# Aikku93/ulc-codec

Hardware: AMD Instinct MI355X
Metric: encode+decode Msamples/s at BlockSize=2048 stereo (channel-samples through encode+decode, VBR -50, 32 blocks per stream per call) (higher is better)
Workload: dtype f32; 1 GPU; vbr50 (configs[1] encode, configs[2] decode): Batch=4096 independent 44.1 kHz stereo streams/GPU x 32 blocks, BlockSize=2048, VBR -50; step = encode then decode; config=vbr50, mode=both, streams_per_gpu=4096, block_size=2048, channels=2, parallelism=batch split over 1 GPU(s), no collective on the data path

## Files before the change

### ulc-codec_amd/csrc/ulcx_enc_wc.hip

```cpp
#include "ulcx_enc_dev.h"

template <typename IN> __device__ __forceinline__ float2 wc_energy_at(const UlcxEncCtx &c, int s, int t) {
    float ehp = 0.0f, ebp = 0.0f;
    if (c.C == 2) {
        float2 a = smp_ld2<IN>(c, s, t - 1), b = smp_ld2<IN>(c, s, t), d = smp_ld2<IN>(c, s, t + 1);
        float m0 = (a.x + a.y) * 0.5f, m1 = (b.x + b.y) * 0.5f, m2 = (d.x + d.y) * 0.5f;
        float s0 = (a.x - a.y) * 0.5f, s1 = (b.x - b.y) * 0.5f, s2 = (d.x - d.y) * 0.5f;
        float hp = -m0 + 2 * m1 - m2, bp = -m0 + m2;
        ehp += hp * hp; ebp += bp * bp;
        hp = -s0 + 2 * s1 - s2; bp = -s0 + s2;
        ehp += hp * hp; ebp += bp * bp;
    } else {
        for (int ch = 0; ch < c.C; ch++) {
            float t0 = ms_sample<IN>(c, s, t - 1, ch), t1 = ms_sample<IN>(c, s, t, ch), t2 = ms_sample<IN>(c, s, t + 1, ch);
            float hp = -t0 + 2 * t1 - t2;
            float bp = -t0 + t2;
            ehp += hp * hp;
            ebp += bp * bp;
        }
    }
    return make_float2(sqrtf(ehp), sqrtf(ebp));
}

template <typename IN>
__global__ __launch_bounds__(WG) void k_wc_energy(UlcxEncCtx c, int k0, int k1) {
    __shared__ float2 tile[64][65];
    int tiles_t = ((k1 - k0) * c.BS) / 64;
    int sg = blockIdx.x / tiles_t, tt = blockIdx.x % tiles_t + (k0 * c.BS) / 64;
    int lane = threadIdx.x & 63, wv = __builtin_amdgcn_readfirstlane(threadIdx.x >> 6);
    int r = tt * 64 + lane;
    int t = r - c.BS / 2;
#pragma unroll 4
    for (int sl = wv; sl < 64; sl += 4) {
        int s = sg * 64 + sl;
        tile[lane][sl] = (s < c.B) ? wc_energy_at<IN>(c, s, t) : make_float2(0.0f, 0.0f);
    }
    __syncthreads();
    float *dst = (float *)c.env + envq_idx(c, sg * 64, tt * 16);
    for (int ql = wv; ql < 16; ql += 4) {
        const float2 a0 = tile[4 * ql][lane], a1 = tile[4 * ql + 1][lane], a2 = tile[4 * ql + 2][lane], a3 = tile[4 * ql + 3][lane];
        float4 *o = (float4 *)(dst + (size_t)ql * 512 + lane * 4);
        wc_st(o, make_float4(a0.x, a1.x, a2.x, a3.x));
        wc_st(o + 64, make_float4(a0.y, a1.y, a2.y, a3.y));
    }
}

__global__ __launch_bounds__(64) void k_wc_forward(UlcxEncCtx c, int k0, int k1) {
    __builtin_amdgcn_s_setprio(3);
    int gl = blockIdx.x * 64 + threadIdx.x;
    int s = gl >> 1, f = gl & 1;
    bool live = s < c.B;
    float4 *v = (float4 *)((float *)c.env + envq_idx(c, live ? s : 0, k0 * c.BS / 4) + f * 256);
    float env = live ? c.wcs[s].tf[f] : 0.0f;
    float cc = f ? c.cBP : c.cHP;
    const int nq = (k1 - k0) * c.BS / 4;
    constexpr int U = 2, D = 8;
    constexpr int QS = 512 / 4;
    const float4 *rp = v;
    float4 *wp = v;
    float4 x[D][U];
#pragma unroll
    for (int g = 0; g < D - 1; g++) {
#pragma unroll
        for (int j = 0; j < U; j++) x[g][j] = wc_ld(rp + (size_t)j * QS);
        rp += U * QS;
    }
    for (int i = 0; i < nq; i += D * U) {
#pragma unroll
        for (int g = 0; g < D; g++) {
            const bool more = (i + (g + D - 1) * U) < nq;
            const float4 *lp = more ? rp : v;
#pragma unroll
            for (int j = 0; j < U; j++) x[(g + D - 1) % D][j] = wc_ld(lp + (size_t)j * QS);
            rp += U * QS;
#pragma unroll
            for (int j = 0; j < U; j++) {
                float4 q = x[g][j];
                float d;
                d = q.x - env; env += d * cc; q.x = env;
                d = q.y - env; env += d * cc; q.y = env;
                d = q.z - env; env += d * cc; q.z = env;
                d = q.w - env; env += d * cc; q.w = env;
                x[g][j] = q;
            }
            if (live) {
#pragma unroll
                for (int j = 0; j < U; j++) wc_st(wp + (size_t)j * QS, x[g][j]);
            }
            wp += U * QS;
        }
    }
    if (live) c.wcs[s].tf[f] = env;
}

__device__ __forceinline__ float2 wc_energy_stereo(float2 a, float2 b, float2 d) {
    float m0 = (a.x + a.y) * 0.5f, m1 = (b.x + b.y) * 0.5f, m2 = (d.x + d.y) * 0.5f;
    float s0 = (a.x - a.y) * 0.5f, s1 = (b.x - b.y) * 0.5f, s2 = (d.x - d.y) * 0.5f;
    float ehp = 0.0f, ebp = 0.0f;
    float hp = -m0 + 2 * m1 - m2, bp = -m0 + m2;
    ehp += hp * hp; ebp += bp * bp;
    hp = -s0 + 2 * s1 - s2; bp = -s0 + s2;
    ehp += hp * hp; ebp += bp * bp;
    return make_float2(sqrtf(ehp), sqrtf(ebp));
}

template <int NW, typename IN>
__global__ __launch_bounds__(NW * 64) void k_wc_ef(UlcxEncCtx c, int k0, int k1) {
    extern __shared__ float efs[];
    float *ring = efs;
    int *flags = (int *)(ring + EF_RT * EF_TILE_FLOATS);
    const int wv = __builtin_amdgcn_readfirstlane(threadIdx.x >> 6), lane = threadIdx.x & 63;
    const int s0 = blockIdx.x * EF_SPW;
    const int nT = (k1 - k0) * c.BS / 64;
    constexpr int NP = NW - 1, NS = (EF_SPW + NP - 1) / NP;
    if (threadIdx.x < NW) flags[threadIdx.x] = 0;
    __syncthreads();
    if (wv > 0) {
        const int p = wv - 1;
        if (p >= EF_SPW) {
            if (lane == 0) __atomic_store_n(&flags[p], 0x7ffffff0, __ATOMIC_RELEASE);
            return;
        }
#ifndef EF_AHEAD
#define EF_AHEAD 3
#endif
        float2 A[EF_AHEAD][NS][3];
        const IN *sbase[NS];
#pragma unroll
        for (int i = 0; i < NS; i++) {
            const int s = s0 + p + NP * i;
            const int sc = ((p + NP * i < EF_SPW) && (s < c.B)) ? s : 0;
            sbase[i] = pcm_base<IN>(c) + (size_t)sc * c.K * c.BS * 2 + 2 * lane;
        }
        auto issue = [&](float2 (&A)[NS][3], int j) {
            const int t0 = (k0 * c.BS + j * 64) - c.BS / 2;
            const int t = t0 + lane;
#pragma unroll
            for (int i = 0; i < NS; i++) {
                const int s = s0 + p + NP * i;
                const bool on = (p + NP * i < EF_SPW) && (s < c.B);
                const int sc = on ? s : 0;
                if (t0 >= 1) {
                    const IN *q = sbase[i] + 2 * (ptrdiff_t)t0;
                    A[i][0] = ld2(q - 2); A[i][1] = ld2(q); A[i][2] = ld2(q + 2);
                } else { A[i][0] = smp_ld2<IN>(c, sc, t - 1); A[i][1] = smp_ld2<IN>(c, sc, t); A[i][2] = smp_ld2<IN>(c, sc, t + 1); }
            }
        };
        auto step = [&](float2 (&A)[NS][3], int j) {
            float2 v[NS];
#pragma unroll
            for (int i = 0; i < NS; i++) v[i] = wc_energy_stereo(A[i][0], A[i][1], A[i][2]);
            if (j + EF_AHEAD < nT) issue(A, j + EF_AHEAD);
            while (j >= __atomic_load_n(&flags[NP], __ATOMIC_ACQUIRE) + EF_RT) __builtin_amdgcn_s_sleep(4);
            float *tile = ring + (j % EF_RT) * EF_TILE_FLOATS;
#pragma unroll
            for (int i = 0; i < NS; i++) {
                const int sl = p + NP * i;
                if (sl < EF_SPW) {
                    const bool on = s0 + sl < c.B;
                    tile[(sl * 2 + 0) * EF_TS + lane] = on ? v[i].x : 0.0f;
                    tile[(sl * 2 + 1) * EF_TS + lane] = on ? v[i].y : 0.0f;
                }
            }
            __builtin_amdgcn_fence(__ATOMIC_RELEASE, "workgroup");
            if (lane == 0) __atomic_store_n(&flags[p], j + 1, __ATOMIC_RELEASE);
        };
#pragma unroll
        for (int a = 0; a < EF_AHEAD; a++) if (a < nT) issue(A[a], a);
        for (int j = 0; j < nT; j += EF_AHEAD) {
#pragma unroll
            for (int a = 0; a < EF_AHEAD; a++) if (j + a < nT) step(A[a], j + a);
        }
        return;
    }
    if (lane >= 2 * EF_SPW) return;
    __builtin_amdgcn_s_setprio(3);
    const int s = s0 + (lane >> 1), f = lane & 1;
    const bool live = s < c.B;
    float env = live ? c.wcs[s].tf[f] : 0.0f;
    const float cc = f ? c.cBP : c.cHP;
    constexpr int QS = 512 / 4;
    char *wq[4];
#pragma unroll
    for (int k = 0; k < 4; k++) wq[k] = (char *)((float *)c.env + envq_idx(c, s, k0 * c.BS / 4) + f * 256) + k * 8192 + 4096;
    for (int j = 0; j < nT; j++) {
        for (;;) {
            int m = (lane < NP) ? __atomic_load_n(&flags[lane], __ATOMIC_ACQUIRE) : 0x7fffffff;
            if (__all(m > j)) break;
            __builtin_amdgcn_s_sleep(1);
        }
        const float4 *row = (const float4 *)(ring + (j % EF_RT) * EF_TILE_FLOATS + lane * EF_TS);
        float4 x[16];
#pragma unroll
        for (int q = 0; q < 16; q++) x[q] = row[q];
        if (lane == 0) __atomic_store_n(&flags[NP], j + 1, __ATOMIC_RELEASE);
#pragma unroll
        for (int q = 0; q < 16; q++) {
            float4 v = x[q];
            float d;
            d = v.x - env; env += d * cc; v.x = env;
            d = v.y - env; env += d * cc; v.y = env;
            d = v.z - env; env += d * cc; v.z = env;
            d = v.w - env; env += d * cc; v.w = env;
            wc_st((float4 *)(wq[q >> 2] + ((q & 3) * 2048 - 4096)), v);
        }
#pragma unroll
        for (int k = 0; k < 4; k++) wq[k] += 16 * QS * sizeof(float4);
    }
    if (live) c.wcs[s].tf[f] = env;
}

__global__ __launch_bounds__(64) void k_wc_backward(UlcxEncCtx c, int k0, int k1) {
    __builtin_amdgcn_s_setprio(3);
    int sl = threadIdx.x;
    int k = k0 + blockIdx.x % (k1 - k0), sg = blockIdx.x / (k1 - k0);
    float *e = (float *)c.env + envq_idx(c, sg * 64 + sl, k * c.BS / 4);
    const int nq = c.BS / 4;
    constexpr int QS = 512 / 4;
    float pHP = e[(size_t)(nq - 1) * 512 + 3], pBP = e[(size_t)(nq - 1) * 512 + 256 + 3];
    const float qHP = c.qHP, qBP = c.qBP;
#ifndef WC_BACK_D
#define WC_BACK_D 4
#endif
    constexpr int U = 2, D = WC_BACK_D;
    const float4 *rp = (const float4 *)(e + (size_t)(nq - 1) * 512);
    float4 *wp = (float4 *)(e + (size_t)(nq - 1) * 512);
    float4 xh[D][U], xb[D][U];
#pragma unroll
    for (int g = 0; g < D - 1; g++) {
#pragma unroll
        for (int j = 0; j < U; j++) { xh[g][j] = wc_ld(rp - (ptrdiff_t)j * QS); xb[g][j] = wc_ld(rp - (ptrdiff_t)j * QS + 64); }
        rp -= U * QS;
    }
    for (int i = 0; i < nq; i += U * D) {
#pragma unroll
        for (int g = 0; g < D; g++) {
            const bool more = (i + (g + D - 1) * U) < nq;
            const float4 *lp = more ? rp : (const float4 *)(e + (size_t)(U - 1) * 512);
#pragma unroll
            for (int j = 0; j < U; j++) { xh[(g + D - 1) % D][j] = wc_ld(lp - (ptrdiff_t)j * QS); xb[(g + D - 1) % D][j] = wc_ld(lp - (ptrdiff_t)j * QS + 64); }
            rp -= U * QS;
            float4 o[U];
#pragma unroll
            for (int j = 0; j < U; j++) {
                const float4 h = xh[g][j], b4 = xb[g][j];
#define WC_BACK_STEP(H, B, O) { float dHP = (H) - pHP, dBP = (B) - pBP; pHP += dHP * qHP; pBP += dBP * qBP; \
                                float a = dHP * pBP, bb = dBP * pHP; (O) = a * a + bb * bb; }
                WC_BACK_STEP(h.w, b4.w, o[j].w) WC_BACK_STEP(h.z, b4.z, o[j].z) WC_BACK_STEP(h.y, b4.y, o[j].y) WC_BACK_STEP(h.x, b4.x, o[j].x)
#undef WC_BACK_STEP
            }
#pragma unroll
            for (int j = 0; j < U; j++) wc_st(wp - (ptrdiff_t)j * QS, o[j]);
            wp -= U * QS;
        }
    }
}

__global__ __launch_bounds__(64) void k_wc_integrate(UlcxEncCtx c, int k0, int k1) {
    __builtin_amdgcn_s_setprio(3);
    int s = blockIdx.x * 64 + threadIdx.x;
    bool live = s < c.B;
    int sc = live ? s : 0;
    float env = c.wcs[sc].tf[2];
    float *bins = c.bins + (size_t)sc * (c.maxK + 1) * 16;
    if (live && k0 == 0) for (int i = 0; i < 8; i++) { bins[i] = c.wcs[s].binSum[i]; bins[8 + i] = c.wcs[s].binW[i]; }
    const float4 *v = (const float4 *)((const float *)c.env + envq_idx(c, s, k0 * c.BS / 4));
    const int bin = c.BS / 8;
    const int nq = (k1 - k0) * c.BS / 4;
#ifndef WC_INT_D
#define WC_INT_D 8
#endif
    constexpr int U = 2, D = WC_INT_D;
    constexpr int QS = 512 / 4;
    const float4 *rp = v;
    float4 x[D][U];
#pragma unroll
    for (int g = 0; g < D - 1; g++) {
#pragma unroll
        for (int j = 0; j < U; j++) x[g][j] = wc_ld(rp + (size_t)j * QS);
        rp += U * QS;
    }
    const float cBlk = c.cBlk;
    float sum = 0.0f;
    int inBin = 0, gbin = k0 * 8;
    auto trip = [&](int i, auto tailT, auto fineT) {
        constexpr bool TAIL = decltype(tailT)::value, FINE = decltype(fineT)::value;
#pragma unroll
        for (int g = 0; g < D; g++) {
            const float4 *lp = rp;
            if (TAIL) { const bool more = (i + (g + D - 1) * U) < nq; lp = more ? rp : v; }
#pragma unroll
            for (int j = 0; j < U; j++) x[(g + D - 1) % D][j] = wc_ld(lp + (size_t)j * QS);
            rp += U * QS;
#pragma unroll
            for (int j = 0; j < U; j++) {
                const float4 q = x[g][j];
                float d;
                d = q.x - env; env += d * cBlk; sum += env;
                d = q.y - env; env += d * cBlk; sum += env;
                d = q.z - env; env += d * cBlk; sum += env;
                d = q.w - env; env += d * cBlk; sum += env;
            }
            if (FINE || g == D - 1) {
                inBin += FINE ? 4 * U : 4 * U * D;
// ... 68 lines not shown
```

### ulc-codec_amd/csrc/ulcx_enc_xf.hip

```cpp
#include "ulcx_enc_dev.h"

__device__ __forceinline__ int first_overlap(int wc, int BS) {
    unsigned p = ulcx_pattern(wc);
    int ov = BS >> (p & 7);
    if (p & 8) ov >>= (wc & 7);
    return ov;
}

__device__ __forceinline__ float win_apply(float x, int i, int S, int aL, int ovL, int aR, int ov,
                                           const float *__restrict__ rise, const float *__restrict__ fall) {
    if (i < S) return (i < aL) ? 0.0f : (i < aL + ovL) ? x * rise[i - aL] : x;
    int n = i - S;
    return (n < aR) ? x : (n < aR + ov) ? x * fall[n - aR] : 0.0f;
}

template <typename IN, int BSC, bool AN = false>
__device__ __forceinline__ int xf_fast(const UlcxEncCtx &c, float *lds, int s, int k, int blk, int tid) {
    constexpr int BS = BSC, S = BSC, M = BSC / 2, PS = 4, Mp = FFT_PADDEDS(M, PS);
    constexpr int LGM = BSC == 4096 ? 11 : 10;
    static_assert(BSC == 2048 || BSC == 4096, "sizes with a compile-time transform");
    static_assert(WG == 256 && (M / 2) % (2 * WG) == 0, "whole fold / epilogue trips per thread");
    float2 *z = (float2 *)lds;
    float2 *twl = (float2 *)(lds + (AN ? 2 : 4) * FFT_PADDEDS(BS, PS));
    float2 *zc0 = z, *zs0 = z + Mp, *zc1 = z + (AN ? 1 : 2) * Mp, *zs1 = z + 3 * Mp;
    const float2 *pre = c.T.pre[0];
    const float *rise = c.T.winRise + S, *fall = c.T.winFall + S;
    const IN *pcmS = pcm_base<IN>(c) + (size_t)s * c.K * BS * 2;
    const IN *frameLo = pcmS + (ptrdiff_t)(k - 2) * BS * 2, *frameHi = frameLo;
    if constexpr (std::is_same<IN, float>::value) {
        const float *histS = c.hist + (size_t)s * 2 * BS * 2;
        if (k < 2) frameLo = histS + (size_t)k * BS * 2;
        if (k < 1) frameHi = histS;
    }
#pragma unroll
    for (int i = tid; i < M / 2; i += WG) twl[i] = c.T.tw[0][i];
#pragma unroll
    for (int jj0 = 0; jj0 < M / 2; jj0 += WG) {
        const int jj = jj0 + tid;
        const int iA = 2 * jj, iB = S - 2 - 2 * jj, iC = S + 2 * jj, iD = 2 * S - 2 - 2 * jj;
        const int ip[4] = { iA, iB, iC, iD };
        float2 xs[8];
#pragma unroll
        for (int r = 0; r < 4; r++) {
            const float4 v = ld4((r < 2 ? frameLo : frameHi) + (size_t)ip[r] * 2);
            const float2 m0 = make_float2((v.x + v.y) * 0.5f, (v.x - v.y) * 0.5f);
            const float2 m1 = make_float2((v.z + v.w) * 0.5f, (v.z - v.w) * 0.5f);
            const float2 fw = (r < 2) ? *(const float2 *)(rise + ip[r]) : *(const float2 *)(fall + ip[r] - S);
            xs[2 * r]     = make_float2(m0.x * fw.x, m0.y * fw.x);
            xs[2 * r + 1] = make_float2(m1.x * fw.y, m1.y * fw.y);
        }
#pragma unroll
        for (int hsel = 0; hsel < 2; hsel++) {
            const int n = hsel ? M / 2 + jj : M / 2 - 1 - jj;
            const float2 lbv = hsel ? xs[0] : xs[1], lav = hsel ? xs[3] : xs[2];
            const float2 rav = hsel ? xs[4] : xs[5], rbv = hsel ? xs[7] : xs[6];
            const float2 P = pre[n];
#pragma unroll
            for (int q = 0; q < 2; q++) {
                const float ra = q ? rav.y : rav.x, rb = q ? rbv.y : rbv.x, la = q ? lav.y : lav.x, lb = q ? lbv.y : lbv.x;
                const float vr = ra + rb, wr = ra - rb;
                const float vl = la - lb, wl = lb + la;
                const float v1 = hsel ? vl : vr, v2 = hsel ? vr : vl;
                const float w1 = hsel ? wl : wr, w2 = hsel ? wr : wl;
                float2 *zc = q ? zc1 : zc0, *zs = q ? zs1 : zs0;
                zc[FFT_PADS(n, PS)] = cmulc(make_float2(v1, v2), P);
                if constexpr (!AN) zs[FFT_PADS(n, PS)] = cmulc(make_float2(w2, w1), P);
            }
        }
    }
    __syncthreads();
    if constexpr (AN) { if (tid < 128) fft_wave_dif_ct<M, PS>(z + __builtin_amdgcn_readfirstlane(tid >> 6) * Mp, twl, tid & 63); }
    else fft_wave_dif_ct<M, PS>(z + __builtin_amdgcn_readfirstlane(tid >> 6) * Mp, twl, tid & 63);
    __syncthreads();
    float *coefO = c.coef + (size_t)blk * (2 * BS);
    constexpr float norm = 2.0f / S;
    int nnz = 0;
    if constexpr (AN) {
#pragma unroll
        for (int e0 = 0; e0 < M / 2; e0 += 2 * WG) {
            const int kA = e0 + 2 * tid, kB = e0 + 2 * tid + 1;
            const int kk2[2] = { kA, kB };
            float re[2][2][4];
#pragma unroll
            for (int u = 0; u < 2; u++) {
                const int k1 = kk2[u], k2 = M - 1 - k1;
                const int r1 = (int)(__brev((unsigned)k1) >> (32 - LGM)), r2 = (int)(__brev((unsigned)k2) >> (32 - LGM));
                const float2 P1 = pre[k1], P2 = pre[k2];
                const fft_v2f Pv1 = { P1.x, P1.y }, Pv2 = { P2.x, P2.y };
#pragma unroll
                for (int q = 0; q < 2; q++) {
                    const float2 *zc = q ? zc1 : zc0;
                    auto cm = [](float2 d, fft_v2f w) { const fft_v2f dv = { d.x, d.y }; const fft_v2f r = fft_cmulc_post_pk(dv, w); return make_float2(r.x, r.y); };
                    const float2 yc1 = cm(zc[FFT_PADS(r1, PS)], Pv1), yc2 = cm(zc[FFT_PADS(r2, PS)], Pv2);
                    const float mdct[4] = { yc1.x, yc2.y, yc2.x, yc1.y };
#pragma unroll
                    for (int p = 0; p < 2; p++) {
                        const int slot = p ? (1 - u) : u;
                        re[q][p][2 * slot] = mdct[2*p] * norm; re[q][p][2 * slot + 1] = mdct[2*p+1] * norm;
                    }
                }
            }
            const int j1 = kA, j2 = M - 1 - kB;
#pragma unroll
            for (int q = 0; q < 2; q++) {
                stnt((float4 *)(coefO + q * BS + 2 * j1), make_float4(re[q][0][0], re[q][0][1], re[q][0][2], re[q][0][3]));
                stnt((float4 *)(coefO + q * BS + 2 * j2), make_float4(re[q][1][0], re[q][1][1], re[q][1][2], re[q][1][3]));
            }
        }
        return 0;
    }
#pragma unroll
    for (int e0 = 0; e0 < M / 2; e0 += 2 * WG) {
        const int kA = e0 + 2 * tid, kB = e0 + 2 * tid + 1;
        const int kk2[2] = { kA, kB };
        float re[2][2][4];
        float ns[2][2][2];
        float am[2][2] = { { 0.0f, 0.0f }, { 0.0f, 0.0f } };
#pragma unroll
        for (int u = 0; u < 2; u++) {
            const int k1 = kk2[u], k2 = M - 1 - k1;
            const int r1 = (int)(__brev((unsigned)k1) >> (32 - LGM)), r2 = (int)(__brev((unsigned)k2) >> (32 - LGM));
            const float2 P1 = pre[k1], P2 = pre[k2];
            const fft_v2f Pv1 = { P1.x, P1.y }, Pv2 = { P2.x, P2.y };
#pragma unroll
            for (int q = 0; q < 2; q++) {
                const float2 *zc = q ? zc1 : zc0, *zs = q ? zs1 : zs0;
                auto cm = [](float2 d, fft_v2f w) { const fft_v2f dv = { d.x, d.y }; const fft_v2f r = fft_cmulc_post_pk(dv, w); return make_float2(r.x, r.y); };
                const float2 yc1 = cm(zc[FFT_PADS(r1, PS)], Pv1), yc2 = cm(zc[FFT_PADS(r2, PS)], Pv2);
                const float2 ys1 = cm(zs[FFT_PADS(r1, PS)], Pv1), ys2 = cm(zs[FFT_PADS(r2, PS)], Pv2);
                const float mdct[4] = { yc1.x, yc2.y, yc2.x, yc1.y };
                const float mdst[4] = { ys1.x, ys2.y, ys2.x, ys1.y };
#pragma unroll
                for (int p = 0; p < 2; p++) {
                    const float re0 = mdct[2*p] * norm,   im0 = mdst[2*p] * norm;
                    const float re1 = mdct[2*p+1] * norm, im1 = mdst[2*p+1] * norm;
                    const float re0s = re0 * re0, im0s = im0 * im0, re1s = re1 * re1, im1s = im1 * im1;
                    const float a0 = re0s + im0s, a1 = re1s + im1s;
                    nnz += (fabsf(re0) < 0.5f * ULCX_COEF_EPS) ? 0 : 1;
                    nnz += (fabsf(re1) < 0.5f * ULCX_COEF_EPS) ? 0 : 1;
                    const int slot = p ? (1 - u) : u;
                    re[q][p][2 * slot] = re0; re[q][p][2 * slot + 1] = re1;
                    ns[q][p][slot] = a0 + a1;
                    am[p][slot] += a0; am[p][slot] += a1;
                }
            }
        }
        const int j1 = kA, j2 = M - 1 - kB;
#pragma unroll
        for (int q = 0; q < 2; q++) {
            stnt((float4 *)(coefO + q * BS + 2 * j1), make_float4(re[q][0][0], re[q][0][1], re[q][0][2], re[q][0][3]));
            stnt((float4 *)(coefO + q * BS + 2 * j2), make_float4(re[q][1][0], re[q][1][1], re[q][1][2], re[q][1][3]));
            stnt((float2 *)(c.nsum + tile_idx(BS / 2, blk * 2 + q, j1)), make_float2(ns[q][0][0], ns[q][0][1]));
            stnt((float2 *)(c.nsum + tile_idx(BS / 2, blk * 2 + q, j2)), make_float2(ns[q][1][0], ns[q][1][1]));
        }
        *(float2 *)(c.amp2 + tile_idx(BS / 2, blk, j1)) = make_float2(am[0][0], am[0][1]);
        *(float2 *)(c.amp2 + tile_idx(BS / 2, blk, j2)) = make_float2(am[1][0], am[1][1]);
    }
    return nnz;
}

template <typename IN>
__device__ __forceinline__ bool xf_is_fast(const UlcxEncCtx &c, int s, int k) {
#ifdef XF_NO_FAST
    return false;
#endif
    const int BS = c.BS;
    const int *wrow = c.wcArr + (size_t)s * (c.maxK + 2) + k;
    const int wcPrev = wrow[0], wc = wrow[1], wcNext = wrow[2];
    if (!(k >= 2 || std::is_same<IN, float>::value) || (ulcx_pattern(wc) >> 4) != 0) return false;
    unsigned pp = ulcx_pattern(wcPrev);
    int lastS = BS;
    do { lastS = BS >> (pp & 7); } while (pp >>= 4);
    int ovFirst = first_overlap(wc, BS);
    if (ovFirst > lastS) ovFirst = lastS;
    return ovFirst == BS && first_overlap(wcNext, BS) >= BS;
}

template <bool ST, typename IN, bool AN = false>
__device__ __forceinline__ void xf_block(const UlcxEncCtx &c, float *lds, int s, int k, const int tid) {
    const int BS = c.BS, C = ST ? 2 : c.C;
    const int blk = s * c.K + k;
    const int ps = ulcx_xf_pad_shift(BS, C);
    float2 *z    = (float2 *)lds;
    constexpr int NA = AN ? 2 : 4;
    float2 *twl  = (float2 *)(lds + NA * FFT_PADDEDS(BS, ps));
    int    &s_nnz = *(int *)(lds + NA * FFT_PADDEDS(BS, ps) + BS / 2);
    const bool ampLds = !AN && (C > 2);
    const bool twInLds = !(ampLds && (size_t)16 * (BS + (BS >> ps)) + (size_t)BS * 4 + 32 > ULCX_LDS_LIMIT);
    float  *amp2 = twInLds ? lds + 4 * FFT_PADDEDS(BS, ps) + BS / 2 + 4 : lds + 4 * FFT_PADDEDS(BS, ps);
    if (!AN && tid == 0) s_nnz = 0;
    if (ampLds) for (int i = tid; i < BS / 2; i += WG) amp2[i] = 0.0f;

    const int *wrow = c.wcArr + (size_t)s * (c.maxK + 2) + k;
    int wcPrev = wrow[0], wc = wrow[1], wcNext = wrow[2];
    if (!AN && c.barkRing && tid == 0 && (ulcx_pattern(wc) & ~8u) != 0) c.decList[atomicAdd(c.decCount, 1)] = blk;
    int nextOv = first_overlap(wcNext, BS);
    int ovFirst;
    {
        unsigned pp = ulcx_pattern(wcPrev);
        int lastS = BS;
        do { lastS = BS >> (pp & 7); } while (pp >>= 4);
        ovFirst = first_overlap(wc, BS);
        if (ovFirst > lastS) ovFirst = lastS;
    }
    size_t cb = (size_t)C * BS;
    float *coefO = c.coef + (size_t)blk * cb;
    int nnz = 0;
    __syncthreads();

#ifdef XF_NO_FAST
    const bool fastBlk = false;
#else
    const bool fastBlk = ST && (BS == 2048 || BS == 4096) && (k >= 2 || std::is_same<IN, float>::value) && (ulcx_pattern(wc) >> 4) == 0
                         && ovFirst == BS && nextOv >= BS;
#endif
    if (fastBlk) nnz = (BS == 2048) ? xf_fast<IN, 2048, AN>(c, lds, s, k, blk, tid) : xf_fast<IN, 4096, AN>(c, lds, s, k, blk, tid);
    else
    for (int ch0 = 0; ch0 < C; ch0 += 2) {
        const int nch = ST ? 2 : ((ch0 + 1 < C) ? 2 : 1);
        unsigned pat = ulcx_pattern(wc);
        int off = 0, ovL = ovFirst;
        do {
            int S = BS >> (pat & 7);
            int d = pat & 7;
            pat >>= 4;
            int ov;
            if (pat) { ov = BS >> (pat & 7); if (pat & 8) ov >>= (wc & 7); }
            else ov = nextOv;
            if (ov > S) ov = S;
            const int M = S >> 1;
            int t0 = (k - 1) * BS - BS / 2 + off - S / 2;
            int aL = (S - ovL) >> 1, aR = (S - ov) >> 1;
            const float *rise = c.T.winRise + ovL, *fall = c.T.winFall + ov;
            const float2 *pre = c.T.pre[d];
            const int Mp = FFT_PADDEDS(M, ps);
            float2 *zc0 = z, *zs0 = z + Mp, *zc1 = z + (AN ? 1 : 2) * Mp, *zs1 = z + 3 * Mp;

            if (twInLds) for (int i = tid; i < M / 2; i += WG) twl[i] = c.T.tw[d][i];
            auto fold = [&](auto inpcmT, auto fullovT) {
                constexpr bool INPCM = decltype(inpcmT)::value, FULLOV = decltype(fullovT)::value;
                const IN *frame = pcm_base<IN>(c) + ((size_t)s * c.K * BS + (INPCM ? t0 : 0)) * C;
                auto ldE = [&](int pos, int e) -> float { return INPCM ? ld1(frame + (size_t)pos * C + e) : smp_ld1<IN>(c, s, t0 + pos, e); };
                auto ldQ = [&](int pos) -> float4 { return INPCM ? ld4(frame + (size_t)pos * C) : smp_ld4<IN>(c, s, t0 + pos); };
                for (int jj = tid; jj < M / 2; jj += WG) {
                    const int iA = 2 * jj, iB = S - 2 - 2 * jj, iC = S + 2 * jj, iD = 2 * S - 2 - 2 * jj;
                    float2 xs[8];
                    {
                        const int ip[4] = { iA, iB, iC, iD };
#pragma unroll
                        for (int r = 0; r < 4; r++) {
                            float2 e0, e1;
                            if (nch == 2) {
                                if (C == 2) { float4 v = ldQ(ip[r]); e0 = make_float2(v.x, v.y); e1 = make_float2(v.z, v.w); }
                                else { e0 = make_float2(ldE(ip[r], ch0), ldE(ip[r], ch0 + 1)); e1 = make_float2(ldE(ip[r] + 1, ch0), ldE(ip[r] + 1, ch0 + 1)); }
                                xs[2 * r]     = make_float2((e0.x + e0.y) * 0.5f, (e0.x - e0.y) * 0.5f);
                                xs[2 * r + 1] = make_float2((e1.x + e1.y) * 0.5f, (e1.x - e1.y) * 0.5f);
                            } else {
                                xs[2 * r] = make_float2(ldE(ip[r], ch0), 0.0f); xs[2 * r + 1] = make_float2(ldE(ip[r] + 1, ch0), 0.0f);
                            }
                        }
                    }
                    const int ipos[8] = { iA, iA + 1, iB, iB + 1, iC, iC + 1, iD, iD + 1 };
#pragma unroll
                    for (int r = 0; r < 8; r++) {
                        if (FULLOV) {
                            float f = (r < 4) ? rise[ipos[r]] : fall[ipos[r] - S];
                            xs[r].x *= f; xs[r].y *= f;
                            continue;
                        }
                        float f; bool zero;
                        if (r < 4) {
                            int idx = ipos[r] - aL;
                            int ci = idx < 0 ? 0 : (idx < ovL ? idx : 0);
                            float tv = rise[ci];
                            f = (idx < ovL) ? tv : 1.0f; zero = idx < 0;
                        } else {
                            int idx = ipos[r] - S - aR;
                            int ci = idx < 0 ? 0 : (idx < ov ? idx : 0);
                            float tv = fall[ci];
                            f = (idx < 0) ? 1.0f : tv; zero = idx >= ov;
                        }
                        float wx = xs[r].x * f, wy = xs[r].y * f;
                        xs[r].x = zero ? 0.0f : wx;
                        xs[r].y = zero ? 0.0f : wy;
                    }
#pragma unroll
                    for (int hsel = 0; hsel < 2; hsel++) {
                        const int n = hsel ? M / 2 + jj : M / 2 - 1 - jj;
                        const float2 lbv = hsel ? xs[0] : xs[1], lav = hsel ? xs[3] : xs[2];
                        const float2 rav = hsel ? xs[4] : xs[5], rbv = hsel ? xs[7] : xs[6];
                        float2 P = pre[n];
#pragma unroll
                        for (int q = 0; q < 2; q++) {
                            if (q >= nch) break;
                            float ra = q ? rav.y : rav.x, rb = q ? rbv.y : rbv.x, la = q ? lav.y : lav.x, lb = q ? lbv.y : lbv.x;
                            float vr = ra + rb, wr = ra - rb;
                            float vl = la - lb, wl = lb + la;
                            float v1 = hsel ? vl : vr, v2 = hsel ? vr : vl;
                            float w1 = hsel ? wl : wr, w2 = hsel ? wr : wl;
                            float2 *zc = q ? zc1 : zc0, *zs = q ? zs1 : zs0;
                            zc[FFT_PADS(n, ps)] = cmulc(make_float2(v1, v2), P);
                            if constexpr (!AN) zs[FFT_PADS(n, ps)] = cmulc(make_float2(w2, w1), P);
                        }
                    }
                }
            };
            if (!(ULCX_DBG(c) & 2)) {
                const bool inPcm = (t0 >= 0), fullOv = (ovL == S) && (ov == S);
                if (inPcm && fullOv) fold(std::true_type{}, std::true_type{});
                else if (inPcm) fold(std::true_type{}, std::false_type{});
                else fold(std::false_type{}, std::false_type{});
            }
            __syncthreads();

            if (!(ULCX_DBG(c) & 1)) for (int a = __builtin_amdgcn_readfirstlane(tid >> 6); a < (AN ? 1 : 2) * nch; a += WG / 64) {
                if (twInLds) fft_wave_dif(z + a * Mp, M, twl, tid & 63, ps);
                else fft_wave_dif(z + a * Mp, M, c.T.tw[d], tid & 63, ps);
            }
            __syncthreads();

            int bits = 31 - __clz(M);
            float norm = 2.0f / S;
            if (!(ULCX_DBG(c) & 4)) for (int kk = tid; kk < M / 2; kk += WG) {
                int k1 = kk, k2 = M - 1 - kk;
                int r1 = (int)(__brev((unsigned)k1) >> (32 - bits));
                int r2 = (int)(__brev((unsigned)k2) >> (32 - bits));
                float2 P1 = pre[k1], P2 = pre[k2];
                float am1 = 0.0f, am2 = 0.0f;
                if (ampLds) { am1 = amp2[off / 2 + k1]; am2 = amp2[off / 2 + k2]; }
#pragma unroll
                for (int q = 0; q < 2; q++) {
                    if (q >= nch) break;
                    int ch = ch0 + q;
                    float2 *zc = q ? zc1 : zc0, *zs = q ? zs1 : zs0;
                    const fft_v2f Pv1 = { P1.x, P1.y }, Pv2 = { P2.x, P2.y };
                    auto cm = [](float2 d, fft_v2f w) { const fft_v2f dv = { d.x, d.y }; const fft_v2f r = fft_cmulc_post_pk(dv, w); return make_float2(r.x, r.y); };
                    float2 yc1 = cm(zc[FFT_PADS(r1, ps)], Pv1), yc2 = cm(zc[FFT_PADS(r2, ps)], Pv2);
                    if constexpr (AN) {
                        const float mdctA[4] = { yc1.x, yc2.y, yc2.x, yc1.y };
#pragma unroll
                        for (int p = 0; p < 2; p++) {
                            const int j = p ? k2 : k1;
                            stnt((float2 *)(coefO + (size_t)ch * BS + off + 2 * j), make_float2(mdctA[2*p] * norm, mdctA[2*p+1] * norm));
                        }
                        continue;
                    }
                    float2 ys1 = cm(zs[FFT_PADS(r1, ps)], Pv1), ys2 = cm(zs[FFT_PADS(r2, ps)], Pv2);
                    float mdct[4] = { yc1.x, yc2.y, yc2.x, yc1.y };
                    float mdst[4] = { ys1.x, ys2.y, ys2.x, ys1.y };
#pragma unroll
                    for (int p = 0; p < 2; p++) {
                        float re0 = mdct[2*p] * norm,   im0 = mdst[2*p] * norm;
                        float re1 = mdct[2*p+1] * norm, im1 = mdst[2*p+1] * norm;
                        float re0s = re0 * re0, im0s = im0 * im0, re1s = re1 * re1, im1s = im1 * im1;
                        float a0 = re0s + im0s, a1 = re1s + im1s;
                        nnz += (fabsf(re0) < 0.5f * ULCX_COEF_EPS) ? 0 : 1;
                        nnz += (fabsf(re1) < 0.5f * ULCX_COEF_EPS) ? 0 : 1;
                        int j = p ? k2 : k1;
                        size_t gi = (size_t)ch * BS + off + 2 * j;
                        stnt((float2 *)(coefO + gi), make_float2(re0, re1));
                        stnt(c.nsum + tile_idx(BS / 2, blk * C + ch, off / 2 + j), a0 + a1);
                        if (p) { am2 += a0; am2 += a1; } else { am1 += a0; am1 += a1; }
                    }
                }
                if (AN) continue;
                if (ampLds) { amp2[off / 2 + k1] = am1; amp2[off / 2 + k2] = am2; }
                else { c.amp2[tile_idx(BS / 2, blk, off / 2 + k1)] = am1; c.amp2[tile_idx(BS / 2, blk, off / 2 + k2)] = am2; }
            }
            __syncthreads();
            off += S; ovL = ov;
        } while (pat);
    }
    if (AN) return;
    for (int o = 32; o > 0; o >>= 1) nnz += __shfl_down(nnz, o);
    if ((tid & 63) == 0) atomicAdd(&s_nnz, nnz);
    if (ampLds) for (int i = tid; i < BS / 2; i += WG) c.amp2[tile_idx(BS / 2, blk, i)] = amp2[i];
    __syncthreads();
    if (tid == 0) c.nnz[blk] = s_nnz;
}

#ifndef ULCX_XF_ANALYSIS_UNIT
template <bool ST, typename IN>
__global__ __launch_bounds__(WG, 4) void k_xf(UlcxEncCtx c, int k0, int k1) {
    extern __shared__ float lds[];
    const int kc = k1 - k0;
    const int NBk = c.B * kc;
    const int per = (NBk + 7) / 8;
    const int vb = (int)(blockIdx.x % 8) * per + (int)(blockIdx.x / 8);
    if (vb >= NBk) return;
    xf_block<ST, IN>(c, lds, vb / kc, k0 + vb % kc, threadIdx.x);
}
#else
template <bool ST, typename IN>
__global__ __launch_bounds__(WG, XFA_LB) void k_xfa(UlcxEncCtx c, int k0, int k1) {
    extern __shared__ float lds[];
    const int kc = k1 - k0;
    const int NBk = c.B * kc;
    const int per = (NBk + 7) / 8;
    const int vb = (int)(blockIdx.x % 8) * per + (int)(blockIdx.x / 8);
    if (vb >= NBk) return;
    xf_block<ST, IN, true>(c, lds, vb / kc, k0 + vb % kc, threadIdx.x);
}
#endif

template <typename IN, bool AN>
__device__ __forceinline__ void xf_big_block(const UlcxEncCtx &c, int k0, int k1) {
    extern __shared__ float lds[];
    const int BS = c.BS, C = c.C;
    const int kc = k1 - k0;
    const int NBk = c.B * kc;
    const int vb = blockIdx.x;
    if (vb >= NBk) return;
    const int s = vb / kc, k = k0 + vb % kc;
    const int blk = s * c.K + k;
    const int tid = threadIdx.x;
    float2 *z = (float2 *)lds;
    __shared__ int s_nnz;
    if (tid == 0) s_nnz = 0;
    const int *wrow = c.wcArr + (size_t)s * (c.maxK + 2) + k;
    const int wcPrev = wrow[0], wc = wrow[1], wcNext = wrow[2];
    if (!AN && c.barkRing && threadIdx.x == 0 && (ulcx_pattern(wc) & ~8u) != 0) c.decList[atomicAdd(c.decCount, 1)] = blk;
    const int nextOv = first_overlap(wcNext, BS);
    int ovFirst;
    {
        unsigned pp = ulcx_pattern(wcPrev);
        int lastS = BS;
        do { lastS = BS >> (pp & 7); } while (pp >>= 4);
        ovFirst = first_overlap(wc, BS);
        if (ovFirst > lastS) ovFirst = lastS;
    }
    const size_t cb = (size_t)C * BS;
    float *coefO = c.coef + (size_t)blk * cb;
    int nnz = 0;
    __syncthreads();
    for (int ch = 0; ch < C; ch++) {
        unsigned pat = ulcx_pattern(wc);
        int off = 0, ovL = ovFirst;
        do {
            const int S = BS >> (pat & 7);
            const int d = pat & 7;
            pat >>= 4;
            int ov;
            if (pat) { ov = BS >> (pat & 7); if (pat & 8) ov >>= (wc & 7); }
            else ov = nextOv;
            if (ov > S) ov = S;
            const int M = S >> 1;
            const int t0 = (k - 1) * BS - BS / 2 + off - S / 2;
            const int aL = (S - ovL) >> 1, aR = (S - ov) >> 1;
            const float *rise = c.T.winRise + ovL, *fall = c.T.winFall + ov;
            const float2 *pre = c.T.pre[d];
            const int bits = 31 - __clz(M);
            const float norm = 2.0f / S;
            for (int kind = 0; kind < (AN ? 1 : 2); kind++) {
                for (int jj = tid; jj < M / 2; jj += WG) {
                    const int iA = 2 * jj, iB = S - 2 - 2 * jj, iC = S + 2 * jj, iD = 2 * S - 2 - 2 * jj;
                    const int ipos[8] = { iA, iA + 1, iB, iB + 1, iC, iC + 1, iD, iD + 1 };
                    float xs[8];
#pragma unroll
                    for (int r = 0; r < 8; r++) xs[r] = win_apply(ms_sample<IN>(c, s, t0 + ipos[r], ch), ipos[r], S, aL, ovL, aR, ov, rise, fall);
#pragma unroll
                    for (int hsel = 0; hsel < 2; hsel++) {
                        const int n = hsel ? M / 2 + jj : M / 2 - 1 - jj;
                        const float lb = hsel ? xs[0] : xs[1], la = hsel ? xs[3] : xs[2];
                        const float ra = hsel ? xs[4] : xs[5], rb = hsel ? xs[7] : xs[6];
                        const float vr = ra + rb, wr = ra - rb;
                        const float vl = la - lb, wl = lb + la;
                        const float v1 = hsel ? vl : vr, v2 = hsel ? vr : vl;
                        const float w1 = hsel ? wl : wr, w2 = hsel ? wr : wl;
                        z[n] = kind ? cmulc(make_float2(w2, w1), pre[n]) : cmulc(make_float2(v1, v2), pre[n]);
                    }
                }
                __syncthreads();
                fftn_dif(z, 1, M, c.T.tw[d], tid);
                for (int kk = tid; kk < M / 2; kk += WG) {
                    const int kA = kk, kB = M - 1 - kk;
                    const int r1 = (int)(__brev((unsigned)kA) >> (32 - bits));
                    const int r2 = (int)(__brev((unsigned)kB) >> (32 - bits));
                    const float2 y1 = cmulc_post(z[r1], pre[kA]), y2 = cmulc_post(z[r2], pre[kB]);
#pragma unroll
                    for (int p = 0; p < 2; p++) {
                        const int j = p ? kB : kA;
                        const size_t gi = (size_t)ch * BS + off + 2 * j;
                        if (kind == 0) {
                            const float m0 = p ? y2.x : y1.x, m1 = p ? y1.y : y2.y;
                            const float re0 = m0 * norm, re1 = m1 * norm;
                            nnz += (fabsf(re0) < 0.5f * ULCX_COEF_EPS) ? 0 : 1;
                            nnz += (fabsf(re1) < 0.5f * ULCX_COEF_EPS) ? 0 : 1;
                            *(float2 *)(coefO + gi) = make_float2(re0, re1);
                        } else {
                            const float m0 = p ? y2.x : y1.x, m1 = p ? y1.y : y2.y;
                            const float im0 = m0 * norm, im1 = m1 * norm;
                            const float2 re = *(const float2 *)(coefO + gi);
                            const float re0s = re.x * re.x, im0s = im0 * im0, re1s = re.y * re.y, im1s = im1 * im1;
                            const float a0 = re0s + im0s, a1 = re1s + im1s;
                            c.nsum[tile_idx(BS / 2, blk * C + ch, off / 2 + j)] = a0 + a1;
                            float *ap = c.amp2 + tile_idx(BS / 2, blk, off / 2 + j);
                            float am = (ch == 0) ? 0.0f : *ap;
                            am += a0; am += a1;
                            *ap = am;
                        }
                    }
                }
                __syncthreads();
            }
            off += S; ovL = ov;
        } while (pat);
    }
    if (AN) return;
    for (int o = 32; o > 0; o >>= 1) nnz += __shfl_down(nnz, o);
    if ((tid & 63) == 0) atomicAdd(&s_nnz, nnz);
    __syncthreads();
    if (tid == 0) c.nnz[blk] = s_nnz;
}

#ifndef ULCX_XF_ANALYSIS_UNIT
template <typename IN>
__global__ __launch_bounds__(WG) void k_xf_big(UlcxEncCtx c, int k0, int k1) {
    xf_big_block<IN, false>(c, k0, k1);
}
#else
template <typename IN>
__global__ __launch_bounds__(WG) void k_xfa_big(UlcxEncCtx c, int k0, int k1) {
    xf_big_block<IN, true>(c, k0, k1);
}
#endif

#ifndef ULCX_XF_ANALYSIS_UNIT
__global__ __launch_bounds__(64) void k_cplx(UlcxEncCtx c, int k0, int k1) {
    const int gidc = blockIdx.x * 64 + threadIdx.x, kcc = k1 - k0;
    if (gidc >= c.B * kcc) return;
    const int blk = (gidc / kcc) * c.K + k0 + gidc % kcc;
    int n = c.C * c.BS;
    const float4 *p = (const float4 *)(c.coef + (size_t)blk * n);
    float cx = 0.0f, cw = 0.0f;
    int tiny = 0;
    auto sums = [&](auto tinyT) {
        constexpr bool TINY = decltype(tinyT)::value;
        for (int i = 0; i < n / 4; i += 4) {
            float4 q[4];
#pragma unroll
            for (int u = 0; u < 4; u++) q[u] = p[i + u];
#pragma unroll
            for (int u = 0; u < 4; u++) {
                float4 v = q[u];
                cx += v.x * v.x; cw += fabsf(v.x);
                cx += v.y * v.y; cw += fabsf(v.y);
                cx += v.z * v.z; cw += fabsf(v.z);
                cx += v.w * v.w; cw += fabsf(v.w);
                if (TINY) {
                    tiny += (fabsf(v.x) >= 0.5f * ULCX_COEF_EPS && fabsf(v.x) < 0x1.0p-29f) ? 1 : 0;
                    tiny += (fabsf(v.y) >= 0.5f * ULCX_COEF_EPS && fabsf(v.y) < 0x1.0p-29f) ? 1 : 0;
                    tiny += (fabsf(v.z) >= 0.5f * ULCX_COEF_EPS && fabsf(v.z) < 0x1.0p-29f) ? 1 : 0;
                    tiny += (fabsf(v.w) >= 0.5f * ULCX_COEF_EPS && fabsf(v.w) < 0x1.0p-29f) ? 1 : 0;
                }
            }
        }
    };
    int mode = c.mode;
    float p0 = c.p0, p1 = c.p1, vbrTarget = c.vbrTarget;
    if (c.rates) {
        const float2 r = c.rates[blk / c.K];
        if (r.x < 0.0f) {
            mode = ULCX_MODE_VBR; p0 = -r.x;
            vbrTarget = 0x1.E4EFB7p3f * ulcx_logf(100.0f / p0);
        } else { mode = (r.y > 0.0f) ? ULCX_MODE_ABR : ULCX_MODE_CBR; p0 = r.x; p1 = r.y; }
        if (__ballot(mode != ULCX_MODE_VBR)) sums(std::true_type{}); else sums(std::false_type{});
    } else if (c.mode == ULCX_MODE_VBR) sums(std::false_type{}); else sums(std::true_type{});
    if (cx != 0.0f) {
        cx = ulcx_logf((cw * cw) / cx) / c.cplxScale;
        if (cx < 0.0f) cx = 0.0f;
        if (cx > 1.0f) cx = 1.0f;
    }
    c.cplx[blk] = cx;
    int maxCoef = c.nnz[blk];
    if (mode == ULCX_MODE_VBR) {
        int nT = maxCoef;
        if (vbrTarget > 0.0f) {
            float ft = (c.C * c.BS) * cx / vbrTarget;
            if (ft < maxCoef) nT = (int)ft;
        }
        c.nout[blk] = nT;
        if (c.rates) {
            c.cbrLo[blk] = 0; c.cbrHi[blk] = maxCoef;
            c.cbrDone[blk] = ULCX_DONE_VBR;
            c.cbrBudget[blk] = 0;
            c.selWin[blk] = make_uint4(0u, 0u, (uint32_t)(c.C * c.BS), 0u);
            for (int u = 0; u < c.C * 4; u++) c.tailSum[((size_t)blk * c.C * 4 + u) * 8 + 6] = 0.0f;
        }
    } else {
        float kbps = p0;
        if (mode == ULCX_MODE_ABR) kbps = p0 * cx / p1;
        int budget = (int)((c.BS * kbps) * 1000.0f / c.rateHz);
        int lo = 0, hi = maxCoef;
        int done = (0 < maxCoef) ? 0 : 1;
        int nOut = (0 < maxCoef) ? (int)((unsigned)(0 + maxCoef) / 2u) : 0;
        while (!done && 4 * (nOut - tiny + 1) > budget) {
            hi = nOut - 1;
            if (!(lo < hi - 1)) { done = 1; nOut = lo; }
            else nOut = (int)((unsigned)(lo + hi) / 2u);
        }
        c.cbrLo[blk] = lo; c.cbrHi[blk] = hi;
        c.cbrDone[blk] = done;
        c.selWin[blk] = make_uint4(0u, 0u, (uint32_t)(c.C * c.BS), 0u);
        for (int u = 0; u < c.C * 4; u++) c.tailSum[((size_t)blk * c.C * 4 + u) * 8 + 6] = 0.0f;
        {
            const unsigned long long open = __ballot(!done);
            if (open && (int)__builtin_amdgcn_mbcnt_hi((uint32_t)(open >> 32), __builtin_amdgcn_mbcnt_lo((uint32_t)open, 0u)) == 0 && !done)
                atomicAdd(c.cbrLive, (int)__popcll(open));
        }
        c.nout[blk] = nOut;
        c.cbrBudget[blk] = budget;
    }
    c.isFb[blk] = 0;
    if (c.useWave) c.slow[blk] = 0;
    if (blk == 0) { *c.fbCount = 0; if (c.useWave) { c.slow[c.B * c.K] = 0; c.slow[c.B * c.K + 1] = 0; } }
    int s = blk / c.K, k = blk % c.K;
    if (c.wcOut)   c.wcOut[blk]   = c.wcArr[(size_t)s * (c.maxK + 2) + k + 1];
    if (c.cplxOut) c.cplxOut[blk] = cx;
}

#else
__global__ __launch_bounds__(64) void k_cplxa(UlcxEncCtx c, int k0, int k1) {
    const int gidc = blockIdx.x * 64 + threadIdx.x, kcc = k1 - k0;
    if (gidc >= c.B * kcc) return;
    const int s = gidc / kcc, k = k0 + gidc % kcc;
    const int blk = s * c.K + k;
    if (c.wcOut) c.wcOut[blk] = c.wcArr[(size_t)s * (c.maxK + 2) + k + 1];
    if (!c.cplxOut) return;
    const int n = c.C * c.BS;
    const float4 *p = (const float4 *)(c.coef + (size_t)blk * n);
    float cx = 0.0f, cw = 0.0f;
    for (int i = 0; i < n / 4; i += 4) {
        float4 q[4];
#pragma unroll
        for (int u = 0; u < 4; u++) q[u] = p[i + u];
#pragma unroll
        for (int u = 0; u < 4; u++) {
            float4 v = q[u];
            cx += v.x * v.x; cw += fabsf(v.x);
            cx += v.y * v.y; cw += fabsf(v.y);
            cx += v.z * v.z; cw += fabsf(v.z);
            cx += v.w * v.w; cw += fabsf(v.w);
        }
    }
    if (cx != 0.0f) {
        cx = ulcx_logf((cw * cw) / cx) / c.cplxScale;
        if (cx < 0.0f) cx = 0.0f;
        if (cx > 1.0f) cx = 1.0f;
    }
    c.cplxOut[blk] = cx;
}
#endif

#ifndef ULCX_XF_ANALYSIS_UNIT
template <typename IN>
__global__ __launch_bounds__(WG) void k_state_update(UlcxEncCtx c) {
    int s = blockIdx.x, tid = threadIdx.x;
    int n = 2 * c.BS * c.C;
    float *h = c.hist + (size_t)s * n;
    int newF = c.K * c.BS * c.C;
    const IN *p = pcm_base<IN>(c) + (size_t)s * newF;
    if (c.K >= 2) {
        for (int i = tid; i < n; i += WG) h[i] = ld1(p + newF - n + i);
    } else {
        int half = n / 2;
        for (int i = tid; i < half; i += WG) { h[i] = h[half + i]; h[half + i] = ld1(p + i); }
    }
    if (tid == 0) {
        UlcxWcState &w = c.wcs[s];
        const int *row = c.wcArr + (size_t)s * (c.maxK + 2);
        w.wcPrev = row[c.K];
        w.wcCur = row[c.K + 1];
        const float *bins = c.bins + ((size_t)s * (c.maxK + 1) + c.K) * 16;
        for (int i = 0; i < 8; i++) { w.binSum[i] = bins[i]; w.binW[i] = bins[8 + i]; }
    }
}

template __global__ void k_xf<false, float>(UlcxEncCtx, int, int);
template __global__ void k_xf<false, int16_t>(UlcxEncCtx, int, int);
template __global__ void k_xf<true, float>(UlcxEncCtx, int, int);
template __global__ void k_xf<true, int16_t>(UlcxEncCtx, int, int);
template __global__ void k_xf_big<float>(UlcxEncCtx, int, int);
template __global__ void k_xf_big<int16_t>(UlcxEncCtx, int, int);
template __global__ void k_state_update<float>(UlcxEncCtx);
template __global__ void k_state_update<int16_t>(UlcxEncCtx);
#else
template __global__ void k_xfa<false, float>(UlcxEncCtx, int, int);
template __global__ void k_xfa<false, int16_t>(UlcxEncCtx, int, int);
template __global__ void k_xfa<true, float>(UlcxEncCtx, int, int);
template __global__ void k_xfa<true, int16_t>(UlcxEncCtx, int, int);
template __global__ void k_xfa_big<float>(UlcxEncCtx, int, int);
template __global__ void k_xfa_big<int16_t>(UlcxEncCtx, int, int);
#endif
```

Before: 55680 Msamples/s.

## Move nonzero count into complexity pass and share neighbor samples via DPP

The transform kernels no longer count nonzero coefficients or do the wave/block reduction and atomics for them. The count is now taken in k_cplx, which already reads every coefficient for its energy sums. Separately, the energy-feature producer loads one stereo sample per lane and gets its left and right neighbours through DPP cross-lane moves. Only edge lanes issue an extra load, which cuts global loads and registers. The trade-off is extra compare work in k_cplx and reliance on DPP row-shift semantics across the 64-lane wave for the edge values.

```diff
diff --git a/ulc-codec_amd/csrc/ulcx_enc_wc.hip b/ulc-codec_amd/csrc/ulcx_enc_wc.hip
--- a/ulc-codec_amd/csrc/ulcx_enc_wc.hip
+++ b/ulc-codec_amd/csrc/ulcx_enc_wc.hip
@@ -93,15 +93,24 @@
     if (live) c.wcs[s].tf[f] = env;
 }
 
-__device__ __forceinline__ float2 wc_energy_stereo(float2 a, float2 b, float2 d) {
-    float m0 = (a.x + a.y) * 0.5f, m1 = (b.x + b.y) * 0.5f, m2 = (d.x + d.y) * 0.5f;
-    float s0 = (a.x - a.y) * 0.5f, s1 = (b.x - b.y) * 0.5f, s2 = (d.x - d.y) * 0.5f;
+__device__ __forceinline__ float2 wc_energy_ms(float m0, float m1, float m2, float s0, float s1, float s2) {
     float ehp = 0.0f, ebp = 0.0f;
     float hp = -m0 + 2 * m1 - m2, bp = -m0 + m2;
     ehp += hp * hp; ebp += bp * bp;
     hp = -s0 + 2 * s1 - s2; bp = -s0 + s2;
     ehp += hp * hp; ebp += bp * bp;
     return make_float2(sqrtf(ehp), sqrtf(ebp));
+}
+__device__ __forceinline__ float wc_from_prev_lane(float own, float edge) {
+    return __int_as_float(__builtin_amdgcn_update_dpp(__float_as_int(edge), __float_as_int(own), 0x138 , 0xf, 0xf, false));
+}
+__device__ __forceinline__ float wc_from_next_lane(float own, float edge) {
+    return __int_as_float(__builtin_amdgcn_update_dpp(__float_as_int(edge), __float_as_int(own), 0x130 , 0xf, 0xf, false));
+}
+__device__ __forceinline__ float2 wc_energy_lanes(float2 b, float2 e) {
+    const float m1 = (b.x + b.y) * 0.5f, s1 = (b.x - b.y) * 0.5f;
+    const float me = (e.x + e.y) * 0.5f, se = (e.x - e.y) * 0.5f;
+    return wc_energy_ms(wc_from_prev_lane(m1, me), m1, wc_from_next_lane(m1, me), wc_from_prev_lane(s1, se), s1, wc_from_next_lane(s1, se));
 }
 
 template <int NW, typename IN>
@@ -124,7 +133,11 @@
 #ifndef EF_AHEAD
 #define EF_AHEAD 3
 #endif
-        float2 A[EF_AHEAD][NS][3];
+        float2 A[EF_AHEAD][NS][2];
+#pragma unroll
+        for (int a = 0; a < EF_AHEAD; a++)
+#pragma unroll
+            for (int i = 0; i < NS; i++) A[a][i][1] = make_float2(0.0f, 0.0f);
         const IN *sbase[NS];
 #pragma unroll
         for (int i = 0; i < NS; i++) {
@@ -132,7 +145,9 @@
             const int sc = ((p + NP * i < EF_SPW) && (s < c.B)) ? s : 0;
             sbase[i] = pcm_base<IN>(c) + (size_t)sc * c.K * c.BS * 2 + 2 * lane;
         }
-        auto issue = [&](float2 (&A)[NS][3], int j) {
+        const bool edgeLane = (lane == 0) || (lane == 63);
+        const int edgeStep = (lane == 0) ? -1 : 1;
+        auto issue = [&](float2 (&A)[NS][2], int j) {
             const int t0 = (k0 * c.BS + j * 64) - c.BS / 2;
             const int t = t0 + lane;
 #pragma unroll
@@ -142,14 +157,18 @@
                 const int sc = on ? s : 0;
                 if (t0 >= 1) {
                     const IN *q = sbase[i] + 2 * (ptrdiff_t)t0;
-                    A[i][0] = ld2(q - 2); A[i][1] = ld2(q); A[i][2] = ld2(q + 2);
-                } else { A[i][0] = smp_ld2<IN>(c, sc, t - 1); A[i][1] = smp_ld2<IN>(c, sc, t); A[i][2] = smp_ld2<IN>(c, sc, t + 1); }
+                    A[i][0] = ld2(q);
+                    if (edgeLane) A[i][1] = ld2(q + 2 * edgeStep);
+                } else {
+                    A[i][0] = smp_ld2<IN>(c, sc, t);
+                    if (edgeLane) A[i][1] = smp_ld2<IN>(c, sc, t + edgeStep);
+                }
             }
         };
-        auto step = [&](float2 (&A)[NS][3], int j) {
+        auto step = [&](float2 (&A)[NS][2], int j) {
             float2 v[NS];
 #pragma unroll
-            for (int i = 0; i < NS; i++) v[i] = wc_energy_stereo(A[i][0], A[i][1], A[i][2]);
+            for (int i = 0; i < NS; i++) v[i] = wc_energy_lanes(A[i][0], A[i][1]);
             if (j + EF_AHEAD < nT) issue(A, j + EF_AHEAD);
             while (j >= __atomic_load_n(&flags[NP], __ATOMIC_ACQUIRE) + EF_RT) __builtin_amdgcn_s_sleep(4);
             float *tile = ring + (j % EF_RT) * EF_TILE_FLOATS;
diff --git a/ulc-codec_amd/csrc/ulcx_enc_xf.hip b/ulc-codec_amd/csrc/ulcx_enc_xf.hip
--- a/ulc-codec_amd/csrc/ulcx_enc_xf.hip
+++ b/ulc-codec_amd/csrc/ulcx_enc_xf.hip
@@ -15,7 +15,7 @@
 }
 
 template <typename IN, int BSC, bool AN = false>
-__device__ __forceinline__ int xf_fast(const UlcxEncCtx &c, float *lds, int s, int k, int blk, int tid) {
+__device__ __forceinline__ void xf_fast(const UlcxEncCtx &c, float *lds, int s, int k, int blk, int tid) {
     constexpr int BS = BSC, S = BSC, M = BSC / 2, PS = 4, Mp = FFT_PADDEDS(M, PS);
     constexpr int LGM = BSC == 4096 ? 11 : 10;
     static_assert(BSC == 2048 || BSC == 4096, "sizes with a compile-time transform");
@@ -74,7 +74,6 @@
     __syncthreads();
     float *coefO = c.coef + (size_t)blk * (2 * BS);
     constexpr float norm = 2.0f / S;
-    int nnz = 0;
     if constexpr (AN) {
 #pragma unroll
         for (int e0 = 0; e0 < M / 2; e0 += 2 * WG) {
@@ -107,7 +106,7 @@
                 stnt((float4 *)(coefO + q * BS + 2 * j2), make_float4(re[q][1][0], re[q][1][1], re[q][1][2], re[q][1][3]));
             }
         }
-        return 0;
+        return;
     }
 #pragma unroll
     for (int e0 = 0; e0 < M / 2; e0 += 2 * WG) {
@@ -136,8 +135,6 @@
                     const float re1 = mdct[2*p+1] * norm, im1 = mdst[2*p+1] * norm;
                     const float re0s = re0 * re0, im0s = im0 * im0, re1s = re1 * re1, im1s = im1 * im1;
                     const float a0 = re0s + im0s, a1 = re1s + im1s;
-                    nnz += (fabsf(re0) < 0.5f * ULCX_COEF_EPS) ? 0 : 1;
-                    nnz += (fabsf(re1) < 0.5f * ULCX_COEF_EPS) ? 0 : 1;
                     const int slot = p ? (1 - u) : u;
                     re[q][p][2 * slot] = re0; re[q][p][2 * slot + 1] = re1;
                     ns[q][p][slot] = a0 + a1;
@@ -156,7 +153,6 @@
         *(float2 *)(c.amp2 + tile_idx(BS / 2, blk, j1)) = make_float2(am[0][0], am[0][1]);
         *(float2 *)(c.amp2 + tile_idx(BS / 2, blk, j2)) = make_float2(am[1][0], am[1][1]);
     }
-    return nnz;
 }
 
 template <typename IN>
@@ -184,11 +180,9 @@
     float2 *z    = (float2 *)lds;
     constexpr int NA = AN ? 2 : 4;
     float2 *twl  = (float2 *)(lds + NA * FFT_PADDEDS(BS, ps));
-    int    &s_nnz = *(int *)(lds + NA * FFT_PADDEDS(BS, ps) + BS / 2);
     const bool ampLds = !AN && (C > 2);
     const bool twInLds = !(ampLds && (size_t)16 * (BS + (BS >> ps)) + (size_t)BS * 4 + 32 > ULCX_LDS_LIMIT);
     float  *amp2 = twInLds ? lds + 4 * FFT_PADDEDS(BS, ps) + BS / 2 + 4 : lds + 4 * FFT_PADDEDS(BS, ps);
-    if (!AN && tid == 0) s_nnz = 0;
     if (ampLds) for (int i = tid; i < BS / 2; i += WG) amp2[i] = 0.0f;
 
     const int *wrow = c.wcArr + (size_t)s * (c.maxK + 2) + k;
@@ -205,7 +199,6 @@
     }
     size_t cb = (size_t)C * BS;
     float *coefO = c.coef + (size_t)blk * cb;
-    int nnz = 0;
     __syncthreads();
 
 #ifdef XF_NO_FAST
@@ -214,7 +207,7 @@
     const bool fastBlk = ST && (BS == 2048 || BS == 4096) && (k >= 2 || std::is_same<IN, float>::value) && (ulcx_pattern(wc) >> 4) == 0
                          && ovFirst == BS && nextOv >= BS;
 #endif
-    if (fastBlk) nnz = (BS == 2048) ? xf_fast<IN, 2048, AN>(c, lds, s, k, blk, tid) : xf_fast<IN, 4096, AN>(c, lds, s, k, blk, tid);
+    if (fastBlk) { if (BS == 2048) xf_fast<IN, 2048, AN>(c, lds, s, k, blk, tid); else xf_fast<IN, 4096, AN>(c, lds, s, k, blk, tid); }
     else
     for (int ch0 = 0; ch0 < C; ch0 += 2) {
         const int nch = ST ? 2 : ((ch0 + 1 < C) ? 2 : 1);
@@ -354,8 +347,6 @@
                         float re1 = mdct[2*p+1] * norm, im1 = mdst[2*p+1] * norm;
                         float re0s = re0 * re0, im0s = im0 * im0, re1s = re1 * re1, im1s = im1 * im1;
                         float a0 = re0s + im0s, a1 = re1s + im1s;
-                        nnz += (fabsf(re0) < 0.5f * ULCX_COEF_EPS) ? 0 : 1;
-                        nnz += (fabsf(re1) < 0.5f * ULCX_COEF_EPS) ? 0 : 1;
                         int j = p ? k2 : k1;
                         size_t gi = (size_t)ch * BS + off + 2 * j;
                         stnt((float2 *)(coefO + gi), make_float2(re0, re1));
@@ -371,12 +362,7 @@
             off += S; ovL = ov;
         } while (pat);
     }
-    if (AN) return;
-    for (int o = 32; o > 0; o >>= 1) nnz += __shfl_down(nnz, o);
-    if ((tid & 63) == 0) atomicAdd(&s_nnz, nnz);
     if (ampLds) for (int i = tid; i < BS / 2; i += WG) c.amp2[tile_idx(BS / 2, blk, i)] = amp2[i];
-    __syncthreads();
-    if (tid == 0) c.nnz[blk] = s_nnz;
 }
 
 #ifndef ULCX_XF_ANALYSIS_UNIT
@@ -415,8 +401,6 @@
     const int blk = s * c.K + k;
     const int tid = threadIdx.x;
     float2 *z = (float2 *)lds;
-    __shared__ int s_nnz;
-    if (tid == 0) s_nnz = 0;
     const int *wrow = c.wcArr + (size_t)s * (c.maxK + 2) + k;
     const int wcPrev = wrow[0], wc = wrow[1], wcNext = wrow[2];
     if (!AN && c.barkRing && threadIdx.x == 0 && (ulcx_pattern(wc) & ~8u) != 0) c.decList[atomicAdd(c.decCount, 1)] = blk;
@@ -431,7 +415,6 @@
     }
     const size_t cb = (size_t)C * BS;
     float *coefO = c.coef + (size_t)blk * cb;
-    int nnz = 0;
     __syncthreads();
     for (int ch = 0; ch < C; ch++) {
         unsigned pat = ulcx_pattern(wc);
@@ -484,8 +467,6 @@
                         if (kind == 0) {
                             const float m0 = p ? y2.x : y1.x, m1 = p ? y1.y : y2.y;
                             const float re0 = m0 * norm, re1 = m1 * norm;
-                            nnz += (fabsf(re0) < 0.5f * ULCX_COEF_EPS) ? 0 : 1;
-                            nnz += (fabsf(re1) < 0.5f * ULCX_COEF_EPS) ? 0 : 1;
                             *(float2 *)(coefO + gi) = make_float2(re0, re1);
                         } else {
                             const float m0 = p ? y2.x : y1.x, m1 = p ? y1.y : y2.y;
@@ -506,11 +487,6 @@
             off += S; ovL = ov;
         } while (pat);
     }
-    if (AN) return;
-    for (int o = 32; o > 0; o >>= 1) nnz += __shfl_down(nnz, o);
-    if ((tid & 63) == 0) atomicAdd(&s_nnz, nnz);
-    __syncthreads();
-    if (tid == 0) c.nnz[blk] = s_nnz;
 }
 
 #ifndef ULCX_XF_ANALYSIS_UNIT
@@ -533,7 +509,7 @@
     int n = c.C * c.BS;
     const float4 *p = (const float4 *)(c.coef + (size_t)blk * n);
     float cx = 0.0f, cw = 0.0f;
-    int tiny = 0;
+    int tiny = 0, nz = 0;
     auto sums = [&](auto tinyT) {
         constexpr bool TINY = decltype(tinyT)::value;
         for (int i = 0; i < n / 4; i += 4) {
@@ -547,6 +523,10 @@
                 cx += v.y * v.y; cw += fabsf(v.y);
                 cx += v.z * v.z; cw += fabsf(v.z);
                 cx += v.w * v.w; cw += fabsf(v.w);
+                nz += (fabsf(v.x) < 0.5f * ULCX_COEF_EPS) ? 0 : 1;
+                nz += (fabsf(v.y) < 0.5f * ULCX_COEF_EPS) ? 0 : 1;
+                nz += (fabsf(v.z) < 0.5f * ULCX_COEF_EPS) ? 0 : 1;
+                nz += (fabsf(v.w) < 0.5f * ULCX_COEF_EPS) ? 0 : 1;
                 if (TINY) {
                     tiny += (fabsf(v.x) >= 0.5f * ULCX_COEF_EPS && fabsf(v.x) < 0x1.0p-29f) ? 1 : 0;
                     tiny += (fabsf(v.y) >= 0.5f * ULCX_COEF_EPS && fabsf(v.y) < 0x1.0p-29f) ? 1 : 0;
@@ -572,7 +552,8 @@
         if (cx > 1.0f) cx = 1.0f;
     }
     c.cplx[blk] = cx;
-    int maxCoef = c.nnz[blk];
+    const int maxCoef = nz;
+    c.nnz[blk] = nz;
     if (mode == ULCX_MODE_VBR) {
         int nT = maxCoef;
         if (vbrTarget > 0.0f) {
```

Result: faster. 56540 Msamples/s, median of 6 (+1.5%).
